# GiulioRomualdi/paper_romualdi_2022_icra_centroidal-mpc-walking

Measured on AMD Instinct MI355X. Metric: centroidal-MPC solves/sec (batch, horizon=20), higher is better.
Workload: dtype f32

## Files before the change

### paper_romualdi_2022_icra_centroidal-mpc-walking_amd/csrc/cmpc_solver.hip

```cpp
#include "cmpc_device.h"

#include <cstdlib>
#include <type_traits>
#include <map>
#include <mutex>

#define NS CMPC_NS
#define NF CMPC_NF
#define NQ CMPC_NQ
#define NU CMPC_NU
#define NXA CMPC_NXA
#define NI CMPC_NI
#define PLD 39
#define GLD 30
#define RLD 36
#define NPAN 46
#define GEO 36
#define SQ_TILE_WAVES 6
#define SQ_SPIN_MAX (1 << 20)
#define SQ_PUB_FLOATS (10 * NPAN * 4 + 128 * 4)
#define ZLD 36
#define MSET (NU * RLD + NPAN * RLD + NS * 16)
#define NTRI 256
#define ID_STRIP_LEN 68
// ... 2 lines not shown
#define DSET_I (3 * NU + 3 * NS + 3)
#define REC_UB 0
#define REC_WT 576
#define REC_ZERO 572
#define REC_N CMPC_REC_N
constexpr int SWEEP_UNROLL = 4;
constexpr int DELTA_UNROLL = 4;

namespace {

#ifdef CMPC_PROFILE
__device__ long long g_prof[128];
__device__ float g_trace[64 * 8];
#define PROF_DECL long long pt_ = __builtin_amdgcn_s_memtime()
#define PROF(slot) do { long long n_ = __builtin_amdgcn_s_memtime(); if (threadIdx.x == 0 && blockIdx.x == 0) g_prof[slot] += n_ - pt_; pt_ = n_; } while (0)
#define PROF2_DECL long long pt2_ = __builtin_amdgcn_s_memtime()
#define PROF3(slot) do { long long n_ = __builtin_amdgcn_s_memtime(); if (threadIdx.x == 192 && blockIdx.x == 0) g_prof[slot] += n_ - pt2_; pt2_ = n_; } while (0)
#define PROF4(slot) do { long long n_ = __builtin_amdgcn_s_memtime(); if (threadIdx.x == 128 && blockIdx.x == 0) g_prof[slot] += n_ - pt2_; pt2_ = n_; } while (0)
#define PROF2(slot) do { long long n_ = __builtin_amdgcn_s_memtime(); if (threadIdx.x == 0 && blockIdx.x == 0) g_prof[slot] += n_ - pt2_; pt2_ = n_; } while (0)
#define PROF5(slot) do { long long n_ = __builtin_amdgcn_s_memtime(); if (threadIdx.x == 216 && blockIdx.x == 0) g_prof[slot] += n_ - pt2_; pt2_ = n_; } while (0)
#define CPROF(i) do { if (ln == 0 && blockIdx.x == 0 && k < N) atomicAdd(reinterpret_cast<unsigned long long*>(&g_prof[32 + 5 * wv + (i)]), (unsigned long long)(__builtin_amdgcn_s_memtime() - pc0_)); } while (0)
#define CPROF2(i) do { if (ln == 0 && blockIdx.x == 0 && k < N) atomicAdd(reinterpret_cast<unsigned long long*>(&g_prof[64 + 8 * wv + (i)]), (unsigned long long)(__builtin_amdgcn_s_memtime() - pc0_)); } while (0)
#ifdef CMPC_PROFILE_LIGHT
#undef PROF2_DECL
#undef PROF2
#undef PROF3
#undef PROF4
#undef PROF5
#undef CPROF
#undef CPROF2
#define CPROF2(i)
#define PROF2_DECL
#define PROF2(slot)
#define PROF3(slot)
#define PROF4(slot)
#define PROF5(slot)
#define CPROF(i)
#define SQPROF_DECL
#define SQPROF(slot)
#else
#define SQPROF_DECL PROF_DECL
#define SQPROF(slot) PROF(slot)
#endif
#else
#define SQPROF_DECL
#define SQPROF(slot)
#define CPROF(i)
#define CPROF2(i)
#define PROF_DECL
#define PROF(slot)
#define PROF2_DECL
#define PROF2(slot)
#define PROF3(slot)
#define PROF4(slot)
#define PROF5(slot)
#endif

struct Ctx {
    CmpcIdx L;
    int N;
    const float* sp;
    float *S, *U, *T, *Z;
    float* LAM;
    float *dS, *dU, *dT, *dZ, *d;
    float *Lf;
    float *geoA;
    float *P0, *Qb, *G, *QuuF, *Pan, *Bval, *Aval, *arow, *ybuf, *fpv, *fpn;
    float *idstrip;
    float *ZT;
    double *QuuD1, *qs1;
    int *Brow, *Arow, *qmask;
    unsigned short* tri;
    double *QuuD, *pv, *pn, *qs, *Pd, *sig, *gco, *redd;
    float* red;
    int* flag;
    int* prog;
};

__device__ inline void wave_lds_sync() { asm volatile("" ::: "memory"); }
typedef __attribute__((address_space(3))) const float* ldsf_t;
typedef __attribute__((address_space(3))) float* ldsw_t;
__device__ inline ldsf_t lds_opaque(const float* p) { ldsf_t q = (ldsf_t)p; asm volatile("" : "+v"(q)); return q; }
__device__ inline ldsw_t lds_opaque_w(float* p) { ldsw_t q = (ldsw_t)p; asm volatile("" : "+v"(q)); return q; }
typedef float v4f __attribute__((ext_vector_type(4)));
typedef float v2f __attribute__((ext_vector_type(2)));
__device__ inline float4 lds_ld4(ldsf_t p)
{
    const v4f v = *reinterpret_cast<__attribute__((address_space(3))) const v4f*>(p);
    return make_float4(v[0], v[1], v[2], v[3]);
}
__device__ inline void lds_ld4x4(ldsf_t p, float4 (&out)[4])
{
    v4f a, b, c, d;
    asm volatile("ds_read_b128 %0, %4\n\tds_read_b128 %1, %4 offset:16\n\tds_read_b128 %2, %4 offset:32\n\tds_read_b128 %3, %4 offset:48\n\ts_waitcnt lgkmcnt(0)"
                 : "=&v"(a), "=&v"(b), "=&v"(c), "=&v"(d)
                 : "v"(p)
                 : "memory");
    out[0] = make_float4(a[0], a[1], a[2], a[3]);
    out[1] = make_float4(b[0], b[1], b[2], b[3]);
    out[2] = make_float4(c[0], c[1], c[2], c[3]);
    out[3] = make_float4(d[0], d[1], d[2], d[3]);
}

typedef unsigned v4u __attribute__((ext_vector_type(4)));
template <bool G>
struct RecRef;
template <>
struct RecRef<false> {
    float* p;
    __device__ RecRef(float* base, int, int k) : p(base + (size_t)REC_N * k) {}
    __device__ float ld(unsigned off) const { return p[off]; }
    __device__ float4 ld4(unsigned off) const { return *reinterpret_cast<const float4*>(p + off); }
    __device__ void st(unsigned off, float v) const { p[off] = v; }
    __device__ void st4(unsigned off, const float4& w) const { *reinterpret_cast<float4*>(p + off) = w; }
};
template <>
struct RecRef<true> {
    typedef __attribute__((address_space(1))) unsigned gu32_t;
    typedef __attribute__((address_space(1))) v4u gv4u_t;
    __amdgpu_buffer_rsrc_t r;
    unsigned so;
    char* gb;
    __device__ RecRef(float* base, int N, int k)
    {
        const unsigned long long a = (unsigned long long)base;
        const unsigned lo = __builtin_amdgcn_readfirstlane((unsigned)a), hi = __builtin_amdgcn_readfirstlane((unsigned)(a >> 32));
        r = __builtin_amdgcn_make_buffer_rsrc((void*)(((unsigned long long)hi << 32) | lo), 0, 4 * REC_N * N, 0x00020000);
        so = 4u * REC_N * (unsigned)k;
        gb = (char*)(((unsigned long long)hi << 32) | lo) + so;
    }
    __device__ float ld(unsigned off) const { return __builtin_bit_cast(float, __builtin_amdgcn_raw_buffer_load_b32(r, 4u * off, so, 0)); }
    __device__ float4 ld4(unsigned off) const
    {
        const v4u v = __builtin_amdgcn_raw_buffer_load_b128(r, 4u * off, so, 0);
        return make_float4(__uint_as_float(v.x), __uint_as_float(v.y), __uint_as_float(v.z), __uint_as_float(v.w));
    }
    __device__ void st(unsigned off, float v) const { *(gu32_t*)(gb + 4u * off) = __float_as_uint(v); }
    __device__ void st4(unsigned off, const float4& w) const
    {
        const v4u v = {__float_as_uint(w.x), __float_as_uint(w.y), __float_as_uint(w.z), __float_as_uint(w.w)};
        *(gv4u_t*)(gb + 4u * off) = v;
    }
};

template <bool FG>
__device__ inline void make_ctx(Ctx& c, char* smem, int N, float* fg_base)
{
    constexpr int KBYTES = (sizeof(CmpcConsts) + 15) & ~15;
    c.L.N = N;
    c.N = N;
    double* dp = reinterpret_cast<double*>(smem + KBYTES);
    c.QuuD = dp; dp += 90;
    c.pv = dp; dp += 40; c.pn = dp; dp += 40; c.qs = dp; dp += 16; c.Pd = dp; dp += 40;
    c.sig = dp; dp += NI; c.gco = dp; dp += NI; dp += 2 * NI;
    c.redd = dp; dp += 8;
    c.QuuD1 = c.QuuD; c.qs1 = c.qs;
    if (!FG) { c.QuuD1 = dp; dp += 90; c.qs1 = dp; dp += 16; }
    float* fp = reinterpret_cast<float*>(dp);
    c.QuuF = fp; fp += NU * RLD;
    c.Pan = fp; fp += NPAN * RLD;
    c.ZT = nullptr;
    if (!FG) {
        c.G = nullptr; c.P0 = nullptr;
        c.Qb = fp; fp += NS * 16;
        fp += MSET;
        c.ZT = fp; fp += SQ_PUB_FLOATS;
// ... 235 lines not shown
}
__device__ inline float amax_nan(float m, float v) { return (v == v) ? fmaxf(m, fabsf(v)) : INFINITY; }
__device__ inline float row_target(float z, float mu_min) { return fmaxf(mu_min * fminf(1.f, z * z), 1e-4f * mu_min); }
__device__ inline float wave_max(float v)
{
    v = fmaxf(v, dpp_f<0xB1>(v));
    v = fmaxf(v, dpp_f<0x4E>(v));
    v = fmaxf(v, dpp_f<0x141>(v));
    v = fmaxf(v, dpp_f<0x140>(v));
    return fmaxf(fmaxf(readlane_f(v, 0), readlane_f(v, 16)), fmaxf(readlane_f(v, 32), readlane_f(v, 48)));
}
__device__ inline double wave_sum(double v)
{
    v += dpp_d<0xB1>(v);
    v += dpp_d<0x4E>(v);
    v += dpp_d<0x141>(v);
    v += dpp_d<0x140>(v);
    return (readlane_d(v, 0) + readlane_d(v, 16)) + (readlane_d(v, 32) + readlane_d(v, 48));
}
template <int NT, int NV>
__device__ inline void block_maxn(float (&v)[NV], float* red, int tid)
{
#pragma unroll
    for (int q = 0; q < NV; ++q) v[q] = wave_max(v[q]);
    __syncthreads();
    if ((tid & 63) == 0) {
#pragma unroll
        for (int q = 0; q < NV; ++q) red[3 * (tid >> 6) + q] = v[q];
    }
    __syncthreads();
#pragma unroll
    for (int q = 0; q < NV; ++q) {
        float r = red[q];
#pragma unroll
        for (int w = 1; w < NT / 64; ++w) r = fmaxf(r, red[3 * w + q]);
        v[q] = uniform_f(r);
    }
}
template <int NT>
__device__ inline double block_sum(double v, double* red, int tid)
{
    v = wave_sum(v);
    __syncthreads();
    if ((tid & 63) == 0) red[tid >> 6] = v;
    __syncthreads();
    double r = red[0];
#pragma unroll
    for (int w = 1; w < NT / 64; ++w) r += red[w];
    return uniform_d(r);
}
template <int NT>
__device__ inline void block_max2_sum(float& m0, float& m1, double& sm, float* red, double* redd, int tid)
{
    m0 = wave_max(m0); m1 = wave_max(m1); sm = wave_sum(sm);
    __syncthreads();
    if ((tid & 63) == 0) { red[3 * (tid >> 6)] = m0; red[3 * (tid >> 6) + 1] = m1; redd[tid >> 6] = sm; }
    __syncthreads();
    float r0 = red[0], r1 = red[1];
    double rs = redd[0];
#pragma unroll
    for (int w = 1; w < NT / 64; ++w) { r0 = fmaxf(r0, red[3 * w]); r1 = fmaxf(r1, red[3 * w + 1]); rs += redd[w]; }
    m0 = uniform_f(r0); m1 = uniform_f(r1); sm = uniform_d(rs);
}

template <int NT>
__device__ inline void all_geo(const Ctx& c, const CmpcConsts& prm, int tid)
{
    for (int e = tid; e < c.N * 24; e += NT) {
        const int k = e / 24, t = e - 24 * k;
        const float* s = c.S + NS * k;
        const int ct = t / 12, j = (t % 12) / 3, i = t % 3;
        const float* R = c.sp + c.L.pR(ct) + 9 * k;
        const float* cn = prm.corners + 12 * ct + 3 * j;
        c.geoA[GEO * k + t] = Rm(R, i, 0) * cn[0] + Rm(R, i, 1) * cn[1] + Rm(R, i, 2) * cn[2] + s[9 + 3 * ct + i] - s[i];
    }
    for (int e = tid; e < c.N * 9; e += NT) {
        const int k = e / 9, t = e - 9 * k, i = t % 3;
        const float* u = c.U + NU * k;
        const float f0 = u[i] + u[3 + i] + u[6 + i] + u[9 + i], f1 = u[12 + i] + u[15 + i] + u[18 + i] + u[21 + i];
        c.geoA[GEO * k + 24 + t] = t < 3 ? f0 : (t < 6 ? f1 : gam_of(c, 0, k) * f0 + gam_of(c, 1, k) * f1);
    }
}

__device__ inline double defect(const Ctx& c, const CmpcConsts& prm, int k, int i)
{
    const float* s = c.S + NS * k;
    const float* u = c.U + NU * k;
    const float* sn = c.S + NS * (k + 1);
    const double dt = prm.dt;
    if (i < 3) return (double)s[i] + dt * (double)s[3 + i] - (double)sn[i];
    if (i < 6) {
        const int a = i - 3;
        double acc = (double)c.sp[c.L.pFext() + 3 * k + a] - (a == 2 ? (double)prm.grav : 0.0);
        for (int ct = 0; ct < 2; ++ct) {
            const float* f = u + 12 * ct;
            acc += (double)gam_of(c, ct, k) * ((double)f[a] + (double)f[3 + a] + (double)f[6 + a] + (double)f[9 + a]);
        }
        return (double)s[i] + dt * acc - (double)sn[i];
    }
    if (i < 9) {
        const int a = i - 6, a1 = (a + 1) % 3, a2 = (a + 2) % 3;
        double tor = (double)c.sp[c.L.pText() + 3 * k + a];
        for (int ct = 0; ct < 2; ++ct) {
            const float* R = c.sp + c.L.pR(ct) + 9 * k;
            const double gam = gam_of(c, ct, k);
            double t = 0.0;
            for (int j = 0; j < 4; ++j) {
                const float* cn = prm.corners + 12 * ct + 3 * j;
                const float* f = u + 12 * ct + 3 * j;
                const double r1 = (double)Rm(R, a1, 0) * cn[0] + (double)Rm(R, a1, 1) * cn[1] + (double)Rm(R, a1, 2) * cn[2]
                                  + (double)s[9 + 3 * ct + a1] - (double)s[a1];
                const double r2 = (double)Rm(R, a2, 0) * cn[0] + (double)Rm(R, a2, 1) * cn[1] + (double)Rm(R, a2, 2) * cn[2]
                                  + (double)s[9 + 3 * ct + a2] - (double)s[a2];
                t += r1 * (double)f[a2] - r2 * (double)f[a1];
            }
            tor += gam * t;
        }
        return (double)s[i] + dt * tor - (double)sn[i];
    }
    {
        const int ct = (i - 9) / 3, a = (i - 9) % 3;
        const float* R = c.sp + c.L.pR(ct) + 9 * k;
        const double gam = gam_of(c, ct, k);
        double land = (double)c.sp[c.L.pNom(ct) + 3 * (k + 1) + a];
        for (int m = 0; m < 3; ++m) land += (double)Rm(R, a, m) * (double)u[24 + 3 * ct + m];
        return gam * (double)s[i] + (1.0 - gam) * land - (double)sn[i];
    }
}

template <typename T>
__device__ inline T Bt_vec(const Ctx& c, const CmpcConsts& prm, int k, int m, const T* v)
{
    const float* geo = c.geoA + GEO * k;
    if (m < 24) {
        const int ct = m / 12, i = m % 3;
        const float* r = geo + 3 * (m / 3);
        const int a1 = (i + 1) % 3, a2 = (i + 2) % 3;
        return (T)prm.dt * (T)gam_of(c, ct, k) * (v[3 + i] + v[6 + a1] * (T)r[a2] - v[6 + a2] * (T)r[a1]);
    }
    const int q = m - 24, ct = q / 3, a = q % 3;
    if (!qfree(c, k, q)) return (T)0;
    const float* R = c.sp + c.L.pR(ct) + 9 * k;
    const T g1 = (T)1 - (T)gam_of(c, ct, k);
    return g1 * ((T)Rm(R, 0, a) * v[9 + 3 * ct] + (T)Rm(R, 1, a) * v[10 + 3 * ct] + (T)Rm(R, 2, a) * v[11 + 3 * ct]);
}

template <typename T>
__device__ inline T At_vec(const Ctx& c, const CmpcConsts& prm, int k, int i, const T* v)
{
    const float* geo = c.geoA + GEO * k;
    const T dt = (T)prm.dt;
    if (i < 3) {
        const int a1 = (i + 1) % 3, a2 = (i + 2) % 3;
        const float* Fs = geo + 30;
        return v[i] + dt * (v[6 + a1] * (T)Fs[a2] - v[6 + a2] * (T)Fs[a1]);
    }
    if (i < 6) return dt * v[i - 3] + v[i];
    if (i < 9) return v[i];
    const int ct = (i - 9) / 3, a = (i - 9) % 3, a1 = (a + 1) % 3, a2 = (a + 2) % 3;
    const float* Fc = geo + 24 + 3 * ct;
    const T gam = (T)gam_of(c, ct, k);
    return gam * (v[i] + dt * ((T)Fc[a1] * v[6 + a2] - (T)Fc[a2] * v[6 + a1]));
}

__device__ inline float AB_step(const Ctx& c, const CmpcConsts& prm, int k, int i, const float* ds, const float* du)
{
    const float* geo = c.geoA + GEO * k;
    const float dt = prm.dt;
    if (i < 3) return ds[i] + dt * ds[3 + i];
    if (i < 6) {
        const int a = i - 3;
        float acc = 0.f;
        for (int ct = 0; ct < 2; ++ct) {
            const float* f = du + 12 * ct;
            acc += gam_of(c, ct, k) * (f[a] + f[3 + a] + f[6 + a] + f[9 + a]);
        }
        return ds[i] + dt * acc;
    }
    if (i < 9) {
        const int a = i - 6, a1 = (a + 1) % 3, a2 = (a + 2) % 3;
        float tor = 0.f;
        for (int ct = 0; ct < 2; ++ct) {
            float t = 0.f;
            const float e1 = ds[9 + 3 * ct + a1] - ds[a1], e2 = ds[9 + 3 * ct + a2] - ds[a2];
#pragma unroll
            for (int j = 0; j < 4; ++j) {
                const float* r = geo + 12 * ct + 3 * j;
                const float* df = du + 12 * ct + 3 * j;
                const float* f = c.U + NU * k + 12 * ct + 3 * j;
                t += r[a1] * df[a2] - r[a2] * df[a1] + e1 * f[a2] - e2 * f[a1];
            }
            tor += gam_of(c, ct, k) * t;
        }
        return ds[i] + dt * tor;
    }
    const int ct = (i - 9) / 3, a = (i - 9) % 3;
    const float* R = c.sp + c.L.pR(ct) + 9 * k;
    const float gam = gam_of(c, ct, k);
    float land = 0.f;
#pragma unroll
    for (int m = 0; m < 3; ++m)
        if (qfree(c, k, 3 * ct + m)) land += Rm(R, a, m) * du[24 + 3 * ct + m];
    return gam * ds[i] + (1.f - gam) * land;
}


__device__ inline double rcp_d(double x)
{
    const double r = (double)__builtin_amdgcn_rcpf((float)x);
    return r * (2.0 - x * r);
// ... 1411 lines not shown
        float dt_ = 0.f, dz_ = 0.f;
        if (row_active(c, k, i)) {
            const float t = c.T[e], z = c.Z[e];
            const float cmu = affine ? 0.f : c.dZ[e];
            const float r = row_val(c, prm, k, i, c.U + NU * k) + t;
            dt_ = -r - row_dot(c, prm, k, i, c.dU + NU * k);
            dz_ = (cmu - z * t) / t - (z / t) * dt_;
        }
        c.dT[e] = dt_; c.dZ[e] = dz_;
    }
    __syncthreads();
}

template <int UNR, bool G>
__device__ __forceinline__ void delta_sweep(const Ctx& c, const CmpcConsts& prm, int tid)
{
    const int N = c.N;
    const int r = tid & 31, half = tid >> 5, blk = r >> 2;
    float* gb = c.ybuf;
    float* lb = c.ybuf + 32;
    float* trash = c.ybuf + 72;
    unsigned loff[16], foff[8];
#pragma unroll
    for (int t = 0; t < 16; ++t) {
        const int mq = half ? (16 + t) >> 2 : t >> 2;
        const int cm = half ? ub_row(16 + t) - 4 * ((16 + t) >> 2) : ub_row(t) - 4 * (t >> 2);
        loff[t] = blk >= mq ? cm + r : REC_ZERO;
    }
    {
        const unsigned ubr = ub_row(r) - 4 * blk, wtr = REC_WT + 32 * (r & 15), r7 = r & 7;
        const unsigned hm = 0u - (unsigned)half, w16 = 0u - (unsigned)(r < 16);
#pragma unroll
        for (int q = 0; q < 8; ++q) {
            const unsigned lo = q >= blk ? ubr + 4 * q : REC_ZERO;
            const unsigned hq = ((wtr + 4 * (q ^ r7)) & w16) | (REC_ZERO & ~w16);
            foff[q] = (lo & ~hm) | (hq & hm);
        }
    }
    const bool hi = half == 1 && r < NS;
    const int j = hi ? r : 0;
    const int ja = j < 3 ? j : (j >= 9 ? (j - 9) % 3 : 0), ja1 = (ja + 1) % 3, ja2 = (ja + 2) % 3;
    const int jct = j >= 12 ? 1 : 0;
    const int gfo = j < 3 ? 30 : 24 + 3 * jct;
    const int je = (j >= 3 && j < 6) ? j - 3 : 0;
    const float him = hi ? 1.f : 0.f;
    const float hposm = (hi && j >= 9) ? 1.f : 0.f, hce = (hi && j >= 3 && j < 6) ? prm.dt : 0.f;
    const float hcg0 = (hi && j < 3) ? prm.dt : 0.f, hcg1 = (hi && j >= 9) ? -prm.dt : 0.f, hjsel = jct ? 1.f : 0.f;
    const bool isF = tid < NF, isQ = tid >= NF && tid < NU;
    const int fi = isF ? tid : 0;
    const int fa = fi % 3, fa1 = (fa + 1) % 3, fa2 = (fa + 2) % 3, fcj = fi / 3;
    const int qq = isQ ? tid - 24 : 0, qct = qq >= 3 ? 1 : 0, qa = qq - 3 * qct;
    const float fsel = (fcj >> 2) ? 1.f : 0.f, qsel = qct ? 1.f : 0.f;
    const float lom = half == 0 ? 1.f : 0.f;
    const float Dm = prm.D[r % 3];
    const float dtc = prm.dt, mu = prm.mu_fr;
    if (tid < NXA) c.fpv[tid] = 0.f;
    if (tid < 32) { gb[tid] = 0.f; }
    wave_lds_sync();
    ldsf_t lp[16];
    ldsf_t fpp[8];
    const int kt = N - 1;
    if (!G) {
#pragma unroll
        for (int t = 0; t < 16; ++t) lp[t] = lds_opaque(c.Lf + (size_t)REC_N * kt + loff[t]);
#pragma unroll
        for (int q = 0; q < 8; ++q) fpp[q] = lds_opaque(c.Lf + (size_t)REC_N * kt + foff[q]);
    }
    ldsf_t wp = lds_opaque(c.dT + NI * kt + 4 * fcj);
    ldsf_t wqp = lds_opaque(c.dT + NI * kt + 32 + qq);
    ldsf_t rfp = lds_opaque(c.sp + c.L.pR(fcj >> 2) + 9 * kt + fa);
    ldsf_t rqp = lds_opaque(c.sp + c.L.pR(qct) + 9 * kt + 3 * qa);
    ldsf_t rr1 = lds_opaque(c.geoA + GEO * kt + 3 * fcj + fa1);
    ldsf_t rr2 = lds_opaque(c.geoA + GEO * kt + 3 * fcj + fa2);
    ldsf_t hf1 = lds_opaque(c.geoA + GEO * kt + gfo + ja1);
    ldsf_t hf2 = lds_opaque(c.geoA + GEO * kt + gfo + ja2);
    ldsf_t gm0 = lds_opaque(c.sp + c.L.pGam(0) + kt);
    ldsf_t gm1 = lds_opaque(c.sp + c.L.pGam(1) + kt);
    typedef __attribute__((address_space(3))) const int* ldsi_t;
    ldsi_t qmp = (ldsi_t)(c.qmask + kt);
    asm volatile("" : "+v"(qmp));
    ldsf_t vN = lds_opaque(c.fpv + NS + fi), v3 = lds_opaque(c.fpv + 3 + fa), v6a = lds_opaque(c.fpv + 6 + fa1), v6b = lds_opaque(c.fpv + 6 + fa2);
    ldsf_t vq = lds_opaque(c.fpv + 9 + 3 * qct);
    ldsf_t hvj = lds_opaque(c.fpv + j), hve = lds_opaque(c.fpv + je), hv1 = lds_opaque(c.fpv + 6 + ja1), hv2 = lds_opaque(c.fpv + 6 + ja2);
    ldsf_t gbp = lds_opaque(gb + 16 * half), lbp = lds_opaque(lb);
    ldsw_t gbs = lds_opaque_w(tid < NU ? gb + tid : trash + (tid & 7));
    ldsw_t lbs = lds_opaque_w(lb + r);
    ldsw_t fps = lds_opaque_w(half == 0 ? (tid < NF ? c.fpv + NS + tid : trash + 8 + (tid & 7)) : (hi ? c.fpv + j : trash + 16 + (tid & 7)));
    ldsw_t lqs = lds_opaque_w((!G && tid < NU) ? c.Lf + (size_t)REC_N * kt + wt_idx(15, tid) : trash + (tid & 7));
    const int lqst = (!G && tid < NU) ? REC_N : 0;
    PROF2_DECL;
    auto stage = [&](int o, int k) {
        float lm[16];
        float4 fm[8];
        if (G) {
            const RecRef<G> rec(c.Lf, N, k);
#pragma unroll
            for (int t = 0; t < 16; ++t) lm[t] = rec.ld(loff[t]);
#pragma unroll
            for (int q = 0; q < 8; ++q) fm[q] = rec.ld4(foff[q]);
        } else {
#pragma unroll
            for (int t = 0; t < 16; ++t) lm[t] = lp[t][REC_N * o];
#pragma unroll
            for (int q = 0; q < 8; ++q) fm[q] = lds_ld4(fpp[q] + REC_N * o);
        }
        const float gam0 = gm0[o], gam1 = gm1[o];
        const float dgam = gam1 - gam0;
        PROF2(24);
        float g;
        {
            const float w0 = wp[NI * o], w1 = wp[NI * o + 1], w2 = wp[NI * o + 2], w3 = wp[NI * o + 3];
            const float wx = w0 - w1 - w2 + w3, wy = w0 + w1 - w2 - w3, ws = w0 + w1 + w2 + w3;
            float gF = rfp[9 * o] * wx + rfp[9 * o + 3] * wy - mu * rfp[9 * o + 6] * ws;
            gF += vN[0] + dtc * fmaf(fsel, dgam, gam0) * (v3[0] + v6a[0] * rr2[GEO * o] - v6b[0] * rr1[GEO * o]);
            const float fr = (float)((qmp[o] >> qq) & 1);
            float gQ = wqp[NI * o] - wqp[NI * o + 6];
            gQ += fr * (1.f - fmaf(qsel, dgam, gam0)) * (rqp[9 * o] * vq[0] + rqp[9 * o + 1] * vq[1] + rqp[9 * o + 2] * vq[2]);
            g = isF ? gF : gQ;
        }
        *gbs = g;
        wave_lds_sync();
        PROF2(25);
        float4 gv[4];
#pragma unroll
        for (int t = 0; t < 4; ++t) gv[t] = lds_ld4(gbp + 4 * t);
        float la, lc;
        {
            v2f lp = v2f{lm[0], lm[1]} * v2f{gv[0].x, gv[0].y}, lq = v2f{lm[2], lm[3]} * v2f{gv[0].z, gv[0].w};
#pragma unroll
            for (int t = 1; t < 4; ++t) {
                lp = __builtin_elementwise_fma(v2f{lm[4 * t], lm[4 * t + 1]}, v2f{gv[t].x, gv[t].y}, lp);
                lq = __builtin_elementwise_fma(v2f{lm[4 * t + 2], lm[4 * t + 3]}, v2f{gv[t].z, gv[t].w}, lq);
            }
            lp += lq;
            la = lp[0]; lc = lp[1];
        }
        const float dl = half_sum(la + lc);
        *lbs = dl;
        if (G) {
            if (tid < NU) { const RecRef<G> rec(c.Lf, N, k); const unsigned lo = wt_idx(15, tid); rec.st(lo, rec.ld(lo) + dl); }
        } else {
            *lqs = *lqs + dl;
            lqs -= lqst;
        }
        wave_lds_sync();
        PROF2(26);
        float4 dv[8];
#pragma unroll
        for (int q = 0; q < 8; ++q) dv[q] = lds_ld4(lbp + 4 * q);
        float sm;
        {
            v2f sp = v2f{fm[0].x, fm[0].y} * v2f{dv[0].x, dv[0].y}, sq = v2f{fm[0].z, fm[0].w} * v2f{dv[0].z, dv[0].w};
#pragma unroll
            for (int q = 1; q < 8; ++q) {
                sp = __builtin_elementwise_fma(v2f{fm[q].x, fm[q].y}, v2f{dv[q].x, dv[q].y}, sp);
                sq = __builtin_elementwise_fma(v2f{fm[q].z, fm[q].w}, v2f{dv[q].z, dv[q].w}, sq);
            }
            sp += sq;
            sm = sp[0] + sp[1];
        }
        const float gamj = fmaf(hjsel, dgam, gam0);
        const float sj = fmaf(hposm, gamj - 1.f, 1.f);
        const float cg = fmaf(hcg1, gamj, hcg0);
        const float hiv = sj * hvj[0] + hce * hve[0] + cg * (hv1[0] * hf2[GEO * o] - hv2[0] * hf1[GEO * o]) - sm;
        const float out = lom * (k > 0 ? Dm : 0.f) * sm + him * hiv;
        wave_lds_sync();
        *fps = out;
        wave_lds_sync();
        PROF2(27);
    };
    auto bump = [&](int n) {
        if (!G) {
#pragma unroll
            for (int t = 0; t < 16; ++t) lp[t] -= REC_N * n;
#pragma unroll
            for (int q = 0; q < 8; ++q) fpp[q] -= REC_N * n;
        }
        wp -= NI * n; wqp -= NI * n; rfp -= 9 * n; rqp -= 9 * n; rr1 -= GEO * n; rr2 -= GEO * n; hf1 -= GEO * n; hf2 -= GEO * n;
        gm0 -= n; gm1 -= n; qmp -= n;
    };
    int k = N - 1;
#pragma unroll 1
    for (; (k + 1) % UNR != 0; --k) {
        stage(0, k);
        bump(1);
    }
#pragma unroll 1
    for (; k >= UNR - 1; k -= UNR) {
        bump(UNR - 1);
#pragma unroll
        for (int i = 0; i < UNR; ++i) stage(UNR - 1 - i, k - i);
        bump(1);
    }
}
template <int UNR, bool G>
__device__ void riccati_delta(const Ctx& c, const CmpcConsts& prm, int tid)
{
    if (tid < 64) delta_sweep<UNR, G>(c, prm, tid);
}

template <int NT>
__device__ void step_lengths(const Ctx& c, int tid, float tau, float& ap, float& ad, int k0 = 0, int k1 = CMPC_NMAX)
{
    float a_p = 1.f, a_d = 1.f;
    const int ke = k1 < c.N ? k1 : c.N;
    for (int e = tid + NI * k0; e < ke * NI; e += NT) {
        const float dt_ = c.dT[e], dz_ = c.dZ[e];
        if (dt_ < 0.f) a_p = fminf(a_p, -tau * c.T[e] / dt_);
        if (dz_ < 0.f) a_d = fminf(a_d, -tau * c.Z[e] / dz_);
    }
    float m[2] = {-a_p, -a_d};
    block_maxn<NT, 2>(m, c.red, tid);
    ap = -m[0]; ad = -m[1];
}

__device__ inline void costate_force_sums(const Ctx& c, int tid, int nth)
{
    const int N = c.N;
    for (int e = tid; e < 9 * N; e += nth) {
        const int k = e / 9, t = e - 9 * k;
        const float* du = c.dU + NU * k;
        const int a = t % 3;
        const float s0 = gam_of(c, 0, k) * (du[a] + du[3 + a] + du[6 + a] + du[9 + a]);
        const float s1 = gam_of(c, 1, k) * (du[12 + a] + du[15 + a] + du[18 + a] + du[21 + a]);
        c.d[NS * k + t] = t < 3 ? s0 : (t < 6 ? s1 : s0 + s1);
    }
}
template <int CTRL>
__device__ inline float dpp_keep(float old, float v) { return __uint_as_float(__builtin_amdgcn_update_dpp(__float_as_uint(old), __float_as_uint(v), CTRL, 0xF, 0xF, false)); }
__device__ inline float lane_next(float v, int lane) { return __int_as_float(__builtin_amdgcn_ds_bpermute(4 * (lane + 1), __float_as_int(v))); }
__device__ inline float suffix_sum(float v, int lane)
{
    v += dpp_f<0x101>(v);
    v += dpp_f<0x102>(v);
    v += dpp_f<0x104>(v);
    v += dpp_f<0x108>(v);
    const float t1 = readlane_f(v, 16), t2 = readlane_f(v, 32), t3 = readlane_f(v, 48);
    const int row = lane >> 4;
    return v + (row == 0 ? t1 + (t2 + t3) : (row == 1 ? t2 + t3 : (row == 2 ? t3 : 0.f)));
}
__device__ inline float suffix_lin(float g, float b, int lane)
{
#define CMPC_LIN_STEP(CT) { const float gn = dpp_keep<CT>(1.f, g), bn = dpp_f<CT>(b); b = fmaf(g, bn, b); g *= gn; }
    CMPC_LIN_STEP(0x101) CMPC_LIN_STEP(0x102) CMPC_LIN_STEP(0x104) CMPC_LIN_STEP(0x108)
#undef CMPC_LIN_STEP
    const int row = lane >> 4;
    const float v48 = readlane_f(b, 48);
    if (row == 2) b = fmaf(g, v48, b);
    const float v32 = readlane_f(b, 32);
    if (row == 1) b = fmaf(g, v32, b);
    const float v16 = readlane_f(b, 16);
    if (row == 0) b = fmaf(g, v16, b);
    return b;
}
template <bool DEFER>
__device__ inline void costate_scan(const Ctx& c, const CmpcConsts& prm, int lane, float ap, bool use_exact, float* vout)
{
    const int N = c.N;
    const bool valid = lane <= N, dyn = lane < N;
    const int k = valid ? lane : N, kd = dyn ? lane : N - 1;
    const float* S = c.S + NS * k;
    const float* dS = c.dS + NS * k;
    const float* geo = c.geoA + GEO * kd;
    const float* dF = c.d + NS * kd;
    const float dtm = dyn ? prm.dt : 0.f;
    const float egm = use_exact ? dtm : 0.f;
    const float on = valid ? 1.f : 0.f;
    float lo[3];
#pragma unroll
    for (int a = 0; a < 3; ++a) lo[a] = c.LAM[NS * (kd + 1) + 6 + a];
    float lold[NS];
    if (!DEFER) {
#pragma unroll
        for (int j = 0; j < NS; ++j) lold[j] = c.LAM[NS * k + j];
    }
// ... 82 lines not shown
__device__ __attribute__((noinline)) void phase_costate(lds_t lds, int Nrt, float* fg_base, float ap, bool exact_in)
{
    CMPC_PHASE_PROLOGUE;
    const bool use_exact = __builtin_amdgcn_readfirstlane((int)exact_in) != 0;
    costate_update(c, prm, tid, ap, use_exact);
}
__device__ inline float dual_extrapolate(float z, float dz) { return fmaxf(z + dz, 0.f); }

template <int NT, int NC, bool FG>
__device__ __attribute__((noinline)) void tail_polish(lds_t lds, int Nrt, float* fg_base, int k0_in, bool duals_in)
{
    CMPC_PHASE_PROLOGUE;
    const int k0 = __builtin_amdgcn_readfirstlane(k0_in);
    const bool duals = __builtin_amdgcn_readfirstlane((int)duals_in) != 0;
    bool last = false, blocked = true;
    for (int pi = 0; pi <= prm.tail_iters + 6 && !last; ++pi) {
        last = pi >= prm.tail_iters + 6 || (pi >= prm.tail_iters && !blocked);
        all_geo<NT>(c, prm, tid);
        for (int e = tid + NS * k0; e < NS * N; e += NT) c.d[e] = (float)defect(c, prm, e / NS, e % NS);
        __syncthreads();
        const float cmu = last ? 0.f : -prm.mu_min;
        int fail = riccati_backward<NT, NC, FG>(lds, c, prm, tid, fg_base, prm.exact_hessian != 0, prm.reg, cmu, k0);
        if (fail) {
            __syncthreads();
            fail = riccati_backward<NT, NC, FG>(lds, c, prm, tid, fg_base, false, prm.reg, cmu, k0);
        }
        if (fail) break;
        if (!last) {
            for (int e = tid + NI * k0; e < NI * N; e += NT) c.dZ[e] = row_active(c, e / NI, e % NI) ? row_target(c.Z[e], prm.mu_min) : 0.f;
            __syncthreads();
        }
        phase_forward_tail<NT, NC, FG>(lds, N, fg_base, last, k0);
        float ap, ad;
        step_lengths<NT>(c, tid, last ? 0.999f : 0.99f, ap, ad, k0);
        float bad = 0.f;
        for (int e = tid + NU * k0; e < NU * N; e += NT) bad = amax_nan(bad, c.dU[e]);
        for (int e = tid + NS * (k0 + 1); e < NS * (N + 1); e += NT) bad = amax_nan(bad, c.dS[e]);
        float m1[1] = {bad};
        block_maxn<NT, 1>(m1, c.red, tid);
        if (!(m1[0] < INFINITY)) break;
        blocked = ap < 0.9f || ad < 0.9f;
        for (int e = tid + NS * (k0 + 1); e < NS * (N + 1); e += NT) c.S[e] += ap * c.dS[e];
        for (int e = tid + NU * k0; e < NU * N; e += NT) c.U[e] += ap * c.dU[e];
        if (!last)
            for (int e = tid + NI * k0; e < NI * N; e += NT) { c.T[e] += ap * c.dT[e]; c.Z[e] += ad * c.dZ[e]; }
        else if (duals)
            for (int e = tid + NI * k0; e < NI * N; e += NT) {
                const float tn = c.T[e] + ap * c.dT[e], zn = dual_extrapolate(c.Z[e], c.dZ[e]);
                if (fabsf(tn) < INFINITY && fabsf(zn) < INFINITY) { c.T[e] = tn; c.Z[e] = zn; }
            }
        __syncthreads();
    }
}

struct Resid { float ep, ec, mu; };
template <int NT, int NC, bool FG>
__device__ __attribute__((noinline)) Resid phase_residuals(lds_t lds, int Nrt, float* fg_base, int nrow_in)
{
    CMPC_PHASE_PROLOGUE;
    const int nrow = __builtin_amdgcn_readfirstlane(nrow_in);
    float l_ep = 0.f, l_ec = 0.f, l_chk = 0.f;
    double l_mu = 0.0;
    all_geo<NT>(c, prm, tid);
    for (int e = tid; e < 24 * N; e += NT) {
        const int k = e / 24, r = e - 24 * k, a = r >> 3, cj = r & 7, ct = cj >> 2;
        const int a1 = (a + 1) % 3, a2 = (a + 2) % 3;
        const float* s = c.S + NS * k;
        const float* f = c.U + NU * k + 3 * cj;
        const float* R = c.sp + c.L.pR(ct) + 9 * k;
        const float* cn = prm.corners + 3 * cj;
        const double r1 = (double)Rm(R, a1, 0) * cn[0] + (double)Rm(R, a1, 1) * cn[1] + (double)Rm(R, a1, 2) * cn[2] + (double)s[9 + 3 * ct + a1] - (double)s[a1];
        const double r2 = (double)Rm(R, a2, 0) * cn[0] + (double)Rm(R, a2, 1) * cn[1] + (double)Rm(R, a2, 2) * cn[2] + (double)s[9 + 3 * ct + a2] - (double)s[a2];
        double t = (double)gam_of(c, ct, k) * (r1 * (double)f[a2] - r2 * (double)f[a1]);
        t += dpp_d<0xB1>(t);
        t += dpp_d<0x4E>(t);
        t += dpp_d<0x141>(t);
        if (cj == 0) {
            const double dv = (double)s[6 + a] + (double)prm.dt * ((double)c.sp[c.L.pText() + 3 * k + a] + t) - (double)c.S[NS * (k + 1) + 6 + a];
            c.d[NS * k + 6 + a] = (float)dv;
            l_ep = fmaxf(l_ep, fabsf((float)dv));
            l_chk += (float)dv;
        }
    }
    for (int e = tid; e < 12 * N; e += NT) {
        const int k = e / 12, ii = e - 12 * k, i = ii < 6 ? ii : ii + 3;
        const double dv = defect(c, prm, k, i);
        c.d[NS * k + i] = (float)dv;
        l_ep = fmaxf(l_ep, fabsf((float)dv));
        l_chk += (float)dv;
    }
    if constexpr (NC > 0) {
        for_slots<0, RowSlots<NT, NC>::R>([&](auto qc) {
            constexpr int q = decltype(qc)::value;
            int e;
            float val, dot;
            const int st = row_slot<NT, NC, q, false>(c, prm, tid, e, val, dot);
            const float t = c.T[e], z = c.Z[e];
            if (st & 2) {
                const float rv = val + t;
                l_ep = fmaxf(l_ep, fabsf(rv));
                l_ec = fmaxf(l_ec, t * z);
                l_chk += rv + t * z;
                l_mu += (double)t * z;
            }
        });
    } else {
        for (int e = tid; e < NI * N; e += NT) {
            const int k = e / NI, i = e % NI;
            if (row_active(c, k, i)) {
                const float t = c.T[e], z = c.Z[e];
                const float rv = row_val(c, prm, k, i, c.U + NU * k) + t;
                l_ep = fmaxf(l_ep, fabsf(rv));
                l_ec = fmaxf(l_ec, t * z);
                l_chk += rv + t * z;
                l_mu += (double)t * z;
            }
        }
    }
    if (!(fabsf(l_chk) < INFINITY)) l_ep = INFINITY;
    block_max2_sum<NT>(l_ep, l_ec, l_mu, c.red, c.redd, tid);
    Resid r;
    r.ep = l_ep; r.ec = l_ec; r.mu = (float)(l_mu / (double)nrow);
    return r;
}

template <int NT, int NC, bool FG>
__device__ __attribute__((noinline)) float phase_update(lds_t lds, int Nrt, float* fg_base, float ap_in, float ad_in)
{
    CMPC_PHASE_PROLOGUE;
    const float ap = uniform_f(ap_in), ad = uniform_f(ad_in);
    for (int e = tid; e < NS * (N + 1); e += NT) c.S[e] += ap * c.dS[e];
    for (int e = tid; e < NU * N; e += NT) c.U[e] += ap * c.dU[e];
    for (int e = tid; e < NI * N; e += NT) {
        const float tn = c.T[e] + ap * c.dT[e];
        float zn = c.Z[e] + ad * c.dZ[e];
        c.T[e] = tn; c.Z[e] = zn;
    }
    float l_st = 0.f, l_sf = 0.f, l_fm = 1.f, l_chk2 = 0.f;
    for (int e = tid; e < NS * (N + 1); e += NT) { const float ds = c.dS[e]; l_st = fmaxf(l_st, fabsf(ds)); l_chk2 += ds; }
    for (int e = tid; e < NU * N; e += NT) {
        const int k = e / NU, m = e % NU;
        const float du = c.dU[e];
        l_chk2 += du;
        if (m < NF) {
            const float* f = c.dU + NU * k + 12 * (m / 12) + m % 3;
            const float mean = 0.25f * (f[0] + f[3] + f[6] + f[9]);
            l_sf = fmaxf(l_sf, fabsf(du - gam_of(c, m / 12, k) * mean));
            if (k > 0) l_sf = fmaxf(l_sf, fabsf(du - c.dU[e - NU]));
            l_fm = fmaxf(l_fm, fabsf(c.U[e]));
        } else l_st = fmaxf(l_st, fabsf(du));
    }
    if (!(fabsf(l_chk2) < INFINITY)) l_st = INFINITY;
    float m3[3] = {l_st, l_sf, l_fm};
    block_maxn<NT, 3>(m3, c.red, tid);
    return ap * fmaxf(m3[0], m3[1] / m3[2]);
}

template <int NT, int NC, bool FG>
__device__ __attribute__((noinline)) bool phase_finish(lds_t lds, int Nrt, float* fg_base, bool duals_in)
{
    CMPC_PHASE_PROLOGUE;
    const bool duals = __builtin_amdgcn_readfirstlane((int)duals_in) != 0;
    float ap, ad;
    step_lengths<NT>(c, tid, 0.999f, ap, ad);
    const int kt = N - prm.tail_stages;
    float l_all = 0.f, l_tail = 0.f, l_fm = 1.f;
    for (int e = tid; e < NS * (N + 1); e += NT) l_all = amax_nan(l_all, c.dS[e]);
    for (int e = tid; e < NU * N; e += NT) {
        const float du = c.dU[e];
        l_all = amax_nan(l_all, du);
        if (e % NU < NF) {
            l_fm = fmaxf(l_fm, fabsf(c.U[e]));
// ... 572 lines not shown
```

Before: 370,300.

## Blend force/foot-row operand pointers in delta sweep and regroup defect evaluation by wave

In the non-G delta sweep, per-lane selected LDS pointers are built once so force and foot-row lanes share one load sequence instead of loading both branches. The fm loads are moved later in the stage, the lqs read is hoisted, and pointer bumps are merged into one per unrolled block. Separately, the defect residual loop is split into per-type helpers and assigned to wave-uniform groups, so each wave evaluates only one defect type without divergence. This adds code complexity and relies on NC/NT shape constraints, with a fallback loop kept for other shapes.

```diff
diff --git a/paper_romualdi_2022_icra_centroidal-mpc-walking_amd/csrc/cmpc_solver.hip b/paper_romualdi_2022_icra_centroidal-mpc-walking_amd/csrc/cmpc_solver.hip
--- a/paper_romualdi_2022_icra_centroidal-mpc-walking_amd/csrc/cmpc_solver.hip
+++ b/paper_romualdi_2022_icra_centroidal-mpc-walking_amd/csrc/cmpc_solver.hip
@@ -108,6 +108,7 @@
 typedef __attribute__((address_space(3))) float* ldsw_t;
 __device__ inline ldsf_t lds_opaque(const float* p) { ldsf_t q = (ldsf_t)p; asm volatile("" : "+v"(q)); return q; }
 __device__ inline ldsw_t lds_opaque_w(float* p) { ldsw_t q = (ldsw_t)p; asm volatile("" : "+v"(q)); return q; }
+__device__ inline ldsf_t lds_opaque_again(ldsf_t q) { asm volatile("" : "+v"(q)); return q; }
 typedef float v4f __attribute__((ext_vector_type(4)));
 typedef float v2f __attribute__((ext_vector_type(2)));
 __device__ inline float4 lds_ld4(ldsf_t p)
@@ -509,22 +510,47 @@
     }
 }
 
-__device__ inline double defect(const Ctx& c, const CmpcConsts& prm, int k, int i)
+__device__ inline double defect_com(const Ctx& c, const CmpcConsts& prm, int k, int a)
+{
+    const float* s = c.S + NS * k;
+    const float* sn = c.S + NS * (k + 1);
+    const double dt = prm.dt;
+    return (double)s[a] + dt * (double)s[3 + a] - (double)sn[a];
+}
+__device__ inline double defect_vel(const Ctx& c, const CmpcConsts& prm, int k, int a)
 {
     const float* s = c.S + NS * k;
     const float* u = c.U + NU * k;
     const float* sn = c.S + NS * (k + 1);
     const double dt = prm.dt;
-    if (i < 3) return (double)s[i] + dt * (double)s[3 + i] - (double)sn[i];
-    if (i < 6) {
-        const int a = i - 3;
-        double acc = (double)c.sp[c.L.pFext() + 3 * k + a] - (a == 2 ? (double)prm.grav : 0.0);
-        for (int ct = 0; ct < 2; ++ct) {
-            const float* f = u + 12 * ct;
-            acc += (double)gam_of(c, ct, k) * ((double)f[a] + (double)f[3 + a] + (double)f[6 + a] + (double)f[9 + a]);
-        }
-        return (double)s[i] + dt * acc - (double)sn[i];
-    }
+    double acc = (double)c.sp[c.L.pFext() + 3 * k + a] - (a == 2 ? (double)prm.grav : 0.0);
+    for (int ct = 0; ct < 2; ++ct) {
+        const float* f = u + 12 * ct;
+        acc += (double)gam_of(c, ct, k) * ((double)f[a] + (double)f[3 + a] + (double)f[6 + a] + (double)f[9 + a]);
+    }
+    return (double)s[3 + a] + dt * acc - (double)sn[3 + a];
+}
+__device__ inline double defect_foot(const Ctx& c, const CmpcConsts& prm, int k, int ct, int a)
+{
+    const float* s = c.S + NS * k;
+    const float* u = c.U + NU * k;
+    const float* sn = c.S + NS * (k + 1);
+    const int i = 9 + 3 * ct + a;
+    const float* R = c.sp + c.L.pR(ct) + 9 * k;
+    const double gam = gam_of(c, ct, k);
+    double land = (double)c.sp[c.L.pNom(ct) + 3 * (k + 1) + a];
+    for (int m = 0; m < 3; ++m) land += (double)Rm(R, a, m) * (double)u[24 + 3 * ct + m];
+    return gam * (double)s[i] + (1.0 - gam) * land - (double)sn[i];
+}
+
+__device__ inline double defect(const Ctx& c, const CmpcConsts& prm, int k, int i)
+{
+    const float* s = c.S + NS * k;
+    const float* u = c.U + NU * k;
+    const float* sn = c.S + NS * (k + 1);
+    const double dt = prm.dt;
+    if (i < 3) return defect_com(c, prm, k, i);
+    if (i < 6) return defect_vel(c, prm, k, i - 3);
     if (i < 9) {
         const int a = i - 6, a1 = (a + 1) % 3, a2 = (a + 2) % 3;
         double tor = (double)c.sp[c.L.pText() + 3 * k + a];
@@ -545,14 +571,7 @@
         }
         return (double)s[i] + dt * tor - (double)sn[i];
     }
-    {
-        const int ct = (i - 9) / 3, a = (i - 9) % 3;
-        const float* R = c.sp + c.L.pR(ct) + 9 * k;
-        const double gam = gam_of(c, ct, k);
-        double land = (double)c.sp[c.L.pNom(ct) + 3 * (k + 1) + a];
-        for (int m = 0; m < 3; ++m) land += (double)Rm(R, a, m) * (double)u[24 + 3 * ct + m];
-        return gam * (double)s[i] + (1.0 - gam) * land - (double)sn[i];
-    }
+    return defect_foot(c, prm, k, (i - 9) / 3, (i - 9) % 3);
 }
 
 template <typename T>
@@ -2130,6 +2149,15 @@
     ldsf_t vN = lds_opaque(c.fpv + NS + fi), v3 = lds_opaque(c.fpv + 3 + fa), v6a = lds_opaque(c.fpv + 6 + fa1), v6b = lds_opaque(c.fpv + 6 + fa2);
     ldsf_t vq = lds_opaque(c.fpv + 9 + 3 * qct);
     ldsf_t hvj = lds_opaque(c.fpv + j), hve = lds_opaque(c.fpv + je), hv1 = lds_opaque(c.fpv + 6 + ja1), hv2 = lds_opaque(c.fpv + 6 + ja2);
+    constexpr bool BLEND = !G && UNR > 1;
+    ldsf_t xa = rfp, xb = rfp, xc = rfp, wa = wp, wb = wp, y0 = vN, y1 = v3, y2 = v6a, y3 = v6b, z1 = rr1, z2 = rr2;
+    if (BLEND) {
+        xa = lds_opaque_again(isF ? rfp : rqp); xb = lds_opaque_again(isF ? rfp + 3 : rqp + 1); xc = lds_opaque_again(isF ? rfp + 6 : rqp + 2);
+        wa = lds_opaque_again(isF ? wp : wqp); wb = lds_opaque_again(isF ? wp + 2 : wqp + 5);
+        y0 = lds_opaque_again(half ? hvj : vN); y1 = lds_opaque_again(half ? hve : (isF ? v3 : vq)); y2 = lds_opaque_again(half ? hv1 : (isF ? v6a : vq + 1));
+        y3 = lds_opaque_again(half ? hv2 : (isF ? v6b : vq + 2));
+        z1 = lds_opaque_again(half ? hf1 : rr1); z2 = lds_opaque_again(half ? hf2 : rr2);
+    }
     ldsf_t gbp = lds_opaque(gb + 16 * half), lbp = lds_opaque(lb);
     ldsw_t gbs = lds_opaque_w(tid < NU ? gb + tid : trash + (tid & 7));
     ldsw_t lbs = lds_opaque_w(lb + r);
@@ -2140,6 +2168,7 @@
     auto stage = [&](int o, int k) {
         float lm[16];
         float4 fm[8];
+        float lq0 = 0.f;
         if (G) {
             const RecRef<G> rec(c.Lf, N, k);
 #pragma unroll
@@ -2149,14 +2178,26 @@
         } else {
 #pragma unroll
             for (int t = 0; t < 16; ++t) lm[t] = lp[t][REC_N * o];
-#pragma unroll
-            for (int q = 0; q < 8; ++q) fm[q] = lds_ld4(fpp[q] + REC_N * o);
+            lq0 = *lqs;
         }
         const float gam0 = gm0[o], gam1 = gm1[o];
         const float dgam = gam1 - gam0;
         PROF2(24);
         float g;
-        {
+        float hy0 = 0.f, hy1 = 0.f, hy2 = 0.f, hy3 = 0.f, hz1 = 0.f, hz2 = 0.f;
+        if (BLEND) {
+            const float w0 = wa[NI * o], w1 = wa[NI * o + 1], w2 = wb[NI * o], w3 = wb[NI * o + 1];
+            const float x1 = xa[9 * o], x2 = xb[9 * o], x3 = xc[9 * o];
+            hy0 = y0[0]; hy1 = y1[0]; hy2 = y2[0]; hy3 = y3[0]; hz1 = z1[GEO * o]; hz2 = z2[GEO * o];
+            const float wx = w0 - w1 - w2 + w3, wy = w0 + w1 - w2 - w3, ws = w0 + w1 + w2 + w3;
+            float gF = x1 * wx + x2 * wy - mu * x3 * ws;
+            gF += hy0 + dtc * fmaf(fsel, dgam, gam0) * (hy1 + hy2 * hz2 - hy3 * hz1);
+            const float fr = (float)((qmp[o] >> qq) & 1);
+            float gQ = w0 - w3;
+            gQ += fr * (1.f - fmaf(qsel, dgam, gam0)) * (x1 * hy1 + x2 * hy2 + x3 * hy3);
+            g = isF ? gF : gQ;
+            asm volatile("" : "+v"(hy0), "+v"(hy1), "+v"(hy2), "+v"(hy3), "+v"(hz1), "+v"(hz2));
+        } else {
             const float w0 = wp[NI * o], w1 = wp[NI * o + 1], w2 = wp[NI * o + 2], w3 = wp[NI * o + 3];
             const float wx = w0 - w1 - w2 + w3, wy = w0 + w1 - w2 - w3, ws = w0 + w1 + w2 + w3;
             float gF = rfp[9 * o] * wx + rfp[9 * o + 3] * wy - mu * rfp[9 * o + 6] * ws;
@@ -2172,6 +2213,10 @@
         float4 gv[4];
 #pragma unroll
         for (int t = 0; t < 4; ++t) gv[t] = lds_ld4(gbp + 4 * t);
+        if (!G) {
+#pragma unroll
+            for (int q = 0; q < 8; ++q) fm[q] = lds_ld4(fpp[q] + REC_N * o);
+        }
         float la, lc;
         {
             v2f lp = v2f{lm[0], lm[1]} * v2f{gv[0].x, gv[0].y}, lq = v2f{lm[2], lm[3]} * v2f{gv[0].z, gv[0].w};
@@ -2188,7 +2233,7 @@
         if (G) {
             if (tid < NU) { const RecRef<G> rec(c.Lf, N, k); const unsigned lo = wt_idx(15, tid); rec.st(lo, rec.ld(lo) + dl); }
         } else {
-            *lqs = *lqs + dl;
+            *lqs = lq0 + dl;
             lqs -= lqst;
         }
         wave_lds_sync();
@@ -2210,7 +2255,8 @@
         const float gamj = fmaf(hjsel, dgam, gam0);
         const float sj = fmaf(hposm, gamj - 1.f, 1.f);
         const float cg = fmaf(hcg1, gamj, hcg0);
-        const float hiv = sj * hvj[0] + hce * hve[0] + cg * (hv1[0] * hf2[GEO * o] - hv2[0] * hf1[GEO * o]) - sm;
+        const float hiv = !BLEND ? sj * hvj[0] + hce * hve[0] + cg * (hv1[0] * hf2[GEO * o] - hv2[0] * hf1[GEO * o]) - sm
+                            : sj * hy0 + hce * hy1 + cg * (hy2 * hz2 - hy3 * hz1) - sm;
         const float out = lom * (k > 0 ? Dm : 0.f) * sm + him * hiv;
         wave_lds_sync();
         *fps = out;
@@ -2224,8 +2270,18 @@
 #pragma unroll
             for (int q = 0; q < 8; ++q) fpp[q] -= REC_N * n;
         }
-        wp -= NI * n; wqp -= NI * n; rfp -= 9 * n; rqp -= 9 * n; rr1 -= GEO * n; rr2 -= GEO * n; hf1 -= GEO * n; hf2 -= GEO * n;
+        if (!BLEND) { wp -= NI * n; wqp -= NI * n; rfp -= 9 * n; rqp -= 9 * n; rr1 -= GEO * n; rr2 -= GEO * n; hf1 -= GEO * n; hf2 -= GEO * n; }
+        else { wa -= NI * n; wb -= NI * n; xa -= 9 * n; xb -= 9 * n; xc -= 9 * n; z1 -= GEO * n; z2 -= GEO * n; }
         gm0 -= n; gm1 -= n; qmp -= n;
+        if (!G) {
+#pragma unroll
+            for (int t = 0; t < 16; ++t) asm volatile("" : "+v"(lp[t]));
+#pragma unroll
+            for (int q = 0; q < 8; ++q) asm volatile("" : "+v"(fpp[q]));
+            if (BLEND) asm volatile("" : "+v"(wa), "+v"(wb), "+v"(xa), "+v"(xb), "+v"(xc), "+v"(z1), "+v"(z2));
+            else asm volatile("" : "+v"(wp), "+v"(wqp), "+v"(rfp), "+v"(rqp), "+v"(rr1), "+v"(rr2), "+v"(hf1), "+v"(hf2));
+            asm volatile("" : "+v"(gm0), "+v"(gm1), "+v"(qmp));
+        }
     };
     int k = N - 1;
 #pragma unroll 1
@@ -2233,12 +2289,22 @@
         stage(0, k);
         bump(1);
     }
+    if (G) {
 #pragma unroll 1
-    for (; k >= UNR - 1; k -= UNR) {
+        for (; k >= UNR - 1; k -= UNR) {
+            bump(UNR - 1);
+#pragma unroll
+            for (int i = 0; i < UNR; ++i) stage(UNR - 1 - i, k - i);
+            bump(1);
+        }
+    } else {
         bump(UNR - 1);
-#pragma unroll
-        for (int i = 0; i < UNR; ++i) stage(UNR - 1 - i, k - i);
-        bump(1);
+#pragma unroll 1
+        for (; k >= UNR - 1; k -= UNR) {
+#pragma unroll
+            for (int i = 0; i < UNR; ++i) stage(UNR - 1 - i, k - i);
+            bump(UNR);
+        }
     }
 }
 template <int UNR, bool G>
@@ -2487,12 +2553,31 @@
             l_chk += (float)dv;
         }
     }
-    for (int e = tid; e < 12 * N; e += NT) {
-        const int k = e / 12, ii = e - 12 * k, i = ii < 6 ? ii : ii + 3;
-        const double dv = defect(c, prm, k, i);
-        c.d[NS * k + i] = (float)dv;
-        l_ep = fmaxf(l_ep, fabsf((float)dv));
-        l_chk += (float)dv;
+    constexpr int LGRP = (3 * NC + 63) / 64 * 64;
+    if constexpr (NC > 0 && !FG && 4 * LGRP <= NT) {
+        static_assert((LGRP & (LGRP - 1)) == 0, "the lane inside a group is taken with a mask");
+        const int tl = tid - (NT - 4 * LGRP);
+        const int grp = __builtin_amdgcn_readfirstlane(tl >= 0 ? tl / LGRP : -1);
+        const int l = tl & (LGRP - 1);
+        if (grp >= 0 && l < 3 * NC) {
+            const int a = (l >= NC ? 1 : 0) + (l >= 2 * NC ? 1 : 0), k = l - NC * a;
+            double dv;
+            int i;
+            if (grp == 0) { i = a; dv = defect_com(c, prm, k, a); }
+            else if (grp == 1) { i = 3 + a; dv = defect_vel(c, prm, k, a); }
+            else { i = 9 + 3 * (grp - 2) + a; dv = defect_foot(c, prm, k, grp - 2, a); }
+            c.d[NS * k + i] = (float)dv;
+            l_ep = fmaxf(l_ep, fabsf((float)dv));
+            l_chk += (float)dv;
+        }
+    } else {
+        for (int e = tid; e < 12 * N; e += NT) {
+            const int k = e / 12, ii = e - 12 * k, i = ii < 6 ? ii : ii + 3;
+            const double dv = ii < 3 ? defect_com(c, prm, k, ii) : (ii < 6 ? defect_vel(c, prm, k, ii - 3) : defect_foot(c, prm, k, ii < 9 ? 0 : 1, ii < 9 ? ii - 6 : ii - 9));
+            c.d[NS * k + i] = (float)dv;
+            l_ep = fmaxf(l_ep, fabsf((float)dv));
+            l_chk += (float)dv;
+        }
     }
     if constexpr (NC > 0) {
         for_slots<0, RowSlots<NT, NC>::R>([&](auto qc) {
```

Result: faster. 374,700, median of 6 (+1.2%).
